# zhaoshan2/pangu-pytorch

Hardware: AMD Instinct MI355X
Metric: forward steps/sec (721x1440x13pl) per MI355X (higher is better)
Workload: dtype f32; 1 GPU; PanguModel fp32 forward, 1 sample/GPU, input (1,5,13,721,1440)+(1,4,721,1440), depths 2-6-6-2, dims 192/384, random-init weights (BASELINE configs[1]); parallelism=dp1

## Files before the change

### include/pangu_hip.h

```cpp
#ifndef PANGU_HIP_H
#define PANGU_HIP_H

#include <stdint.h>

#ifdef __cplusplus
extern "C" {
#endif

#define PANGU_ABI_VERSION 1

#define PANGU_OK 0
#define PANGU_E_SHAPE (-1)
#define PANGU_E_NULL (-2)
#define PANGU_E_DTYPE (-3)
#define PANGU_E_ARG (-4)
#define PANGU_E_RANGE (-5)

#define PANGU_F32 0
#define PANGU_BF16 1

#define PANGU_ACT_NONE 0
#define PANGU_ACT_GELU 1
#define PANGU_ACT_GELU_BWD 2
#define PANGU_ACT_ADD 3
#define PANGU_ACT_GELU_BWD_H 4

typedef void* pangu_stream_t;

int pangu_abi_version(void);
const char* pangu_error_string(int code);


int pangu_window_index_export(pangu_stream_t stream, int32_t* out, int Z, int H, int W, int shifted);

int pangu_window_mask_export(pangu_stream_t stream, float* out, int Z, int H, int W);


int pangu_linear_fwd(pangu_stream_t stream, const float* A, int lda, const float* W, const float* bias,
                     float* C, int ldc, int M, int N, int K, int act, float* aux);

int pangu_split_weight_bf16x3(pangu_stream_t stream, const float* W, int N, int K, void* image);
int pangu_linear_fwd_split(pangu_stream_t stream, const float* A, int lda, const void* image, const float* bias,
                           float* C, int ldc, int M, int N, int K, int act);

int pangu_linear_wgrad(pangu_stream_t stream, const float* dC, int lddc, const float* A, int lda, float* dW,
                       float* db, int M, int N, int K);
int pangu_linear_wgrad_ws(pangu_stream_t stream, const float* dC, int lddc, const float* A, int lda, float* dW,
                          float* db, int M, int N, int K, float* workspace, long long workspace_bytes);


int pangu_lora_wgrad_f32(pangu_stream_t stream, const float* dY, int lddy, const float* X, int ldx, const float* A,
                         const float* B, float* dA, float* dB, int M, int N, int K, int r, float scaling, float* workspace,
                         long long workspace_bytes);
int pangu_lora_wgrad_bf16(pangu_stream_t stream, const void* dY, int lddy, const void* X, int ldx, const float* A, const float* B,
                          float* dA, float* dB, int M, int N, int K, int r, float scaling, float* workspace,
                          long long workspace_bytes);
int pangu_lora_merge_f32(pangu_stream_t stream, const float* W, const float* A, const float* B, float* W_eff, int N, int K,
                         int r, float scaling);


int pangu_lora_dropout_fwd_f32(pangu_stream_t stream, const float* X, int ldx, float* Y, int ldy, const float* A, const float* B,
                               int M, int N, int K, int r, float scaling, double p, unsigned seed, int act, float* H, int ldh);
int pangu_lora_wgrad_dropout_f32(pangu_stream_t stream, const float* dY, int lddy, const float* X, int ldx, const float* A,
                                 const float* B, float* dA, float* dB, float* V, int M, int N, int K, int r, float scaling, double p,
                                 unsigned seed, float* workspace, long long workspace_bytes);
int pangu_lora_dropout_dx_f32(pangu_stream_t stream, float* dX, int lddx, const float* V, const float* A, int M, int K, int r,
                              double p, unsigned seed, const float* pre, int ldpre);


int pangu_lora_dropout_fwd_bf16(pangu_stream_t stream, const void* X, int ldx, void* Y, int ldy, const float* A, const float* B,
                                int M, int N, int K, int r, float scaling, double p, unsigned seed, int act, void* H, int ldh);
int pangu_lora_wgrad_dropout_bf16(pangu_stream_t stream, const void* dY, int lddy, const void* X, int ldx, const float* A,
                                  const float* B, float* dA, float* dB, float* V, int M, int N, int K, int r, float scaling, double p,
                                  unsigned seed, float* workspace, long long workspace_bytes);
int pangu_lora_dropout_dx_bf16(pangu_stream_t stream, void* dX, int lddx, const float* V, const float* A, int M, int K, int r,
                               double p, unsigned seed, const void* pre, int ldpre);


int pangu_window_attn_fwd(pangu_stream_t stream, const float* qkv, const float* qkv_bias, const float* esb,
                          float* out, float* lse, int Z, int H, int W, int C, int heads, int shifted);
int pangu_window_attn_fwd_compact(pangu_stream_t stream, const float* qkv, const float* qkv_bias,
                                  const float* esb_compact, float* out, float* lse, int Z, int H, int W, int C,
                                  int heads, int shifted);

int pangu_attn_windows_fwd(pangu_stream_t stream, const float* qkv, const float* esb, const float* mask,
                           long long mask_lon_stride, float* out, int n_lon, int types, int heads, int C);

int pangu_attn_windows_bwd(pangu_stream_t stream, const float* qkv, const float* esb, const float* mask,
                           long long mask_lon_stride, const float* dout, float* dqkv, float* d_esb, int n_lon, int types,
                           int heads, int C);

int pangu_window_attn_bwd(pangu_stream_t stream, const float* qkv, const float* qkv_bias, const float* esb,
                          const float* out, const float* lse, const float* dout, float* dqkv, float* dqkv_bias,
                          float* d_esb, int Z, int H, int W, int C, int heads, int shifted);


int pangu_ln_residual_fwd(pangu_stream_t stream, const float* y, const float* shortcut, int lds,
                          const float* gamma, const float* beta, float* out, int ldo, float* mean_rstd,
                          int N, int C, float branch_scale);

int pangu_linear_ln_residual_fwd(pangu_stream_t stream, const float* A, int lda, const float* W, const float* bias,
                                 const float* shortcut, int lds, const float* gamma, const float* beta, float* out, int ldo,
                                 int M, int N, int K, float branch_scale);

int pangu_linear_ln_residual_fwd_split(pangu_stream_t stream, const float* A, int lda, const void* image, const float* bias,
                                       const float* shortcut, int lds, const float* gamma, const float* beta, float* out,
                                       int ldo, int M, int N, int K, float branch_scale);

int pangu_ln_residual_bwd(pangu_stream_t stream, const float* dout, int lddo, const float* y, const float* gamma,
                          float* dy, float* dgamma, float* dbeta, int N, int C, float branch_scale);

int pangu_downsample_ln_fwd(pangu_stream_t stream, const float* x, int ldx, const float* gamma,
                            const float* beta, float* out, float* mean_rstd, int Z, int H, int W, int C);

int pangu_downsample_ln_bwd(pangu_stream_t stream, const float* dout, const float* x, int ldx, const float* gamma,
                            float* dx, float* dgamma, float* dbeta, int Z, int H, int W, int C, const float* dx_add);

int pangu_upsample_ln_fwd(pangu_stream_t stream, const float* y, const float* gamma, const float* beta,
                          float* out, float* mean_rstd, int Z, int H2, int W2, int H, int Co);

int pangu_upsample_ln_bwd(pangu_stream_t stream, const float* dout, const float* y, const float* gamma, float* dy,
                          float* dgamma, float* dbeta, int Z, int H2, int W2, int H, int Co);


int pangu_patch_embed_gather(pangu_stream_t stream, const float* input, const float* input_surface,
                             const float* surface_mean, const float* surface_std, const float* upper_mean,
                             const float* upper_std, const float* maps, const float* const_h,
                             float* a_surface, float* a_upper, int LAT, int LON, int levels_reversed);

int pangu_patch_embed_gather_bwd(pangu_stream_t stream, const float* da_surface, const float* da_upper,
                                 const float* surface_std, const float* upper_std, float* d_input,
                                 float* d_input_surface, int LAT, int LON, int levels_reversed);

int pangu_patch_recover_scatter(pangu_stream_t stream, const float* y_upper, const float* y_surface,
                                float* output, float* output_surface, int LAT, int LON);
int pangu_patch_recover_scatter_denorm(pangu_stream_t stream, const float* y_upper, const float* y_surface, float* output,
                                       float* output_surface, float* phys, float* phys_surface, const float* upper_mean,
                                       const float* upper_std, const float* surface_mean, const float* surface_std, int LAT,
                                       int LON);

int pangu_patch_recover_gather_bwd(pangu_stream_t stream, const float* d_output, const float* d_output_surface,
                                   float* dy_upper, float* dy_surface, int LAT, int LON);


int pangu_lat_weighted_sums(pangu_stream_t stream, const float* pred, const float* target, const float* lat_weight,
                            float* out, int planes, int H, int W);


int pangu_ensemble_perturb_f32(pangu_stream_t stream, float* upper, long long upper_member_stride, float* surface,
                               long long surface_member_stride, int E, int first_member, int H, int W, const float* amplitude,
                               const float* upper_std, const float* surface_std, unsigned int seed, int octaves, int period,
                               float persistence, int control);

int pangu_ensemble_stats_f32(pangu_stream_t stream, const float* members, long long member_stride, int E, const float* target,
                             const float* clim, const float* lat_weight, float* out, float* mean_out, float* std_out,
                             float* workspace, long long workspace_bytes, int planes, int H, int W);

int pangu_ensemble_reliability_f32(pangu_stream_t stream, const float* members, long long member_stride, int E,
                                   const float* target, const float* thresholds, int T, const float* lat_weight,
                                   unsigned int seed, int first_plane, unsigned int* counts, float* freq, float* prob,
                                   void* workspace, long long workspace_bytes, int planes, int H, int W);

long long pangu_ensemble_quantiles_ws_bytes(int planes, int H, int Q);
int pangu_ensemble_quantiles_f32(pangu_stream_t stream, const float* members, long long member_stride, int E,
                                 const double* levels, int Q, const float* target, const float* lat_weight, float* fields,
                                 float* pinball, unsigned int* coverage_count, float* coverage_freq, unsigned int* nonfinite,
// ... 139 lines not shown
```

### pangu-pytorch_amd/_lib.py

```python
import ctypes
import os
import re

_HERE = os.path.dirname(os.path.abspath(__file__))
LIB_PATH = os.environ.get("PANGU_HIP_LIB") or os.path.join(_HERE, "libpangu_hip.so")
HEADER_PATH = os.path.join(os.path.dirname(_HERE), "include", "pangu_hip.h")

_c = ctypes
_P, _I, _F = _c.c_void_p, _c.c_int, _c.c_float

SIGNATURES = {
    "pangu_abi_version": [],
    "pangu_error_string": [_I],
    "pangu_window_index_export": [_P, _P, _I, _I, _I, _I],
    "pangu_window_mask_export": [_P, _P, _I, _I, _I],
    "pangu_linear_fwd": [_P, _P, _I, _P, _P, _P, _I, _I, _I, _I, _I, _P],
    "pangu_split_weight_bf16x3": [_P, _P, _I, _I, _P],
    "pangu_linear_fwd_split": [_P, _P, _I, _P, _P, _P, _I, _I, _I, _I, _I],
    "pangu_linear_wgrad": [_P, _P, _I, _P, _I, _P, _P, _I, _I, _I],
    "pangu_linear_wgrad_ws": [_P, _P, _I, _P, _I, _P, _P, _I, _I, _I, _P, _c.c_longlong],
    "pangu_lora_wgrad_f32": [_P, _P, _I, _P, _I, _P, _P, _P, _P, _I, _I, _I, _I, _F, _P, _c.c_longlong],
    "pangu_lora_wgrad_bf16": [_P, _P, _I, _P, _I, _P, _P, _P, _P, _I, _I, _I, _I, _F, _P, _c.c_longlong],
    "pangu_lora_merge_f32": [_P, _P, _P, _P, _P, _I, _I, _I, _F],
    "pangu_lora_dropout_fwd_f32": [_P, _P, _I, _P, _I, _P, _P, _I, _I, _I, _I, _F, _c.c_double, _c.c_uint, _I, _P, _I],
    "pangu_lora_wgrad_dropout_f32": [_P, _P, _I, _P, _I, _P, _P, _P, _P, _P, _I, _I, _I, _I, _F, _c.c_double, _c.c_uint, _P,
                                     _c.c_longlong],
    "pangu_lora_dropout_dx_f32": [_P, _P, _I, _P, _P, _I, _I, _I, _c.c_double, _c.c_uint, _P, _I],
    "pangu_lora_dropout_fwd_bf16": [_P, _P, _I, _P, _I, _P, _P, _I, _I, _I, _I, _F, _c.c_double, _c.c_uint, _I, _P, _I],
    "pangu_lora_wgrad_dropout_bf16": [_P, _P, _I, _P, _I, _P, _P, _P, _P, _P, _I, _I, _I, _I, _F, _c.c_double, _c.c_uint, _P,
                                      _c.c_longlong],
    "pangu_lora_dropout_dx_bf16": [_P, _P, _I, _P, _P, _I, _I, _I, _c.c_double, _c.c_uint, _P, _I],
    "pangu_window_attn_bwd": [_P] * 10 + [_I] * 6,
    "pangu_ln_residual_bwd": [_P, _P, _I, _P, _P, _P, _P, _P, _I, _I, _F],
    "pangu_downsample_ln_bwd": [_P, _P, _P, _I, _P, _P, _P, _P, _I, _I, _I, _I, _P],
    "pangu_upsample_ln_bwd": [_P, _P, _P, _P, _P, _P, _P, _I, _I, _I, _I, _I],
    "pangu_patch_recover_gather_bwd": [_P, _P, _P, _P, _P, _I, _I],
    "pangu_lat_weighted_sums": [_P, _P, _P, _P, _P, _I, _I, _I],
    "pangu_ensemble_perturb_f32": [_P, _P, _c.c_longlong, _P, _c.c_longlong, _I, _I, _I, _I, _P, _P, _P, _c.c_uint, _I, _I, _F, _I],
    "pangu_ensemble_stats_f32": [_P, _P, _c.c_longlong, _I, _P, _P, _P, _P, _P, _P, _P, _c.c_longlong, _I, _I, _I],
    "pangu_ensemble_reliability_f32": [_P, _P, _c.c_longlong, _I, _P, _P, _I, _P, _c.c_uint, _I, _P, _P, _P, _P, _c.c_longlong, _I, _I,
                                       _I],
    "pangu_ensemble_quantiles_ws_bytes": [_I, _I, _I],
    "pangu_ensemble_quantiles_f32": [_P, _P, _c.c_longlong, _I, _P, _I, _P, _P, _P, _P, _P, _P, _P, _P, _c.c_longlong, _I, _I, _I],
    "pangu_zonal_spectrum_ws_bytes": [_I, _I, _I, _I, _I],
    "pangu_zonal_spectrum_f32": [_P, _P, _c.c_longlong, _I, _P, _P, _I, _P, _P, _I, _P, _P, _c.c_longlong, _I, _I, _I],
    "pangu_linear_fwd_bf16": [_P, _P, _I, _P, _P, _P, _I, _I, _I, _I, _I, _P, _I],
    "pangu_window_attn_fwd_bf16": [_P, _P, _P, _P, _P, _P, _I, _I, _I, _I, _I, _I],
    "pangu_window_attn_qkv_fwd_bf16": [_P, _P, _I, _P, _P, _P, _P, _P, _I, _I, _I, _I, _I, _I],
    "pangu_ln_residual_fwd_bf16": [_P, _P, _P, _I, _P, _P, _P, _I, _I, _I, _F],
    "pangu_linear_ln_residual_fwd_bf16": [_P, _P, _I, _P, _P, _P, _P, _P, _P, _I, _I, _I, _I],
    "pangu_mlp_ln_residual_fwd_bf16": [_P, _P, _I, _P, _P, _P, _P, _P, _P, _I, _I, _I, _F],
    "pangu_mlp_ln_residual_train_fwd_bf16": [_P, _P, _I, _P, _P, _P, _P, _P, _P, _I, _P, _I, _P, _I, _I, _I, _F],
    "pangu_linear_gelu_bwd_bf16": [_P, _P, _I, _P, _P, _I, _I, _I, _I, _P, _P],
    "pangu_downsample_ln_fwd_bf16": [_P, _P, _I, _P, _P, _P, _I, _I, _I, _I],
    "pangu_upsample_ln_fwd_bf16": [_P, _P, _P, _P, _P, _I, _I, _I, _I, _I],
    "pangu_patch_embed_gather_bf16": [_P] * 11 + [_I, _I, _I],
    "pangu_linear_wgrad_bf16": [_P, _P, _I, _P, _I, _P, _P, _I, _I, _I],
    "pangu_linear_wgrad_bf16_ws": [_P, _P, _I, _P, _I, _P, _P, _I, _I, _I, _P, _c.c_longlong],
    "pangu_shadow_refresh_bf16": [_P, _P, _I, _c.c_longlong],
    "pangu_adam_step_multi": [_P, _P, _I, _c.c_longlong] + [_c.c_double] * 5 + [_F, _F],
    "pangu_grad_sumsq_multi": [_P, _P, _I, _c.c_longlong, _P],
    "pangu_grad_clip_state": [_P, _P, _c.c_longlong, _P, _I, _c.c_double, _c.c_double, _I],
    "pangu_adam_step_multi_scaled": [_P, _P, _I, _c.c_longlong] + [_c.c_double] * 5 + [_F, _F, _P],
    "pangu_weighted_l1_loss_blocks": [_I, _I, _c.c_longlong, _I, _c.c_longlong, _I],
    "pangu_weighted_l1_loss_fwd": [_P] * 9 + [_I, _I, _c.c_longlong, _I, _c.c_longlong, _I, _I] + [_P] * 4,
    "pangu_weighted_l1_loss_bwd": [_P] * 10 + [_I, _I, _c.c_longlong, _I, _c.c_longlong, _I, _I] + [_P] * 4,
    "pangu_rollout_l1_seed_bwd": [_P] * 14 + [_I, _I, _c.c_longlong, _I, _c.c_longlong, _I, _I] + [_P] * 4,
    "pangu_fair_crps_loss_blocks": [_I] * 7,
    "pangu_fair_crps_loss_fwd": [_P, _P, _P, _I] + [_P] * 7 + [_I] * 7 + [_P] * 4,
    "pangu_fair_crps_loss_bwd": [_P, _P, _P, _I] + [_P] * 8 + [_I] * 7 + [_P] * 4,
    "pangu_host_copy": [_P, _P, _c.c_longlong, _I],
    "pangu_pack_i16_ws_bytes": [_I, _c.c_longlong],
    "pangu_pack_planes_i16": [_P, _P, _P, _P, _P, _P, _P, _P, _c.c_longlong, _I, _c.c_longlong, _I],
    "pangu_stage_planes_f32": [_P, _P, _P, _P, _P, _I, _c.c_longlong, _I],
    "pangu_unpack_i16_host": [_P, _P, _P, _I, _c.c_longlong, _I],
    "pangu_regrid_planes_f32": [_P, _P, _P, _P, _P, _I, _I, _I, _I, _I, _P, _P, _P, _I, _P, _P, _P, _I, _I],
    "pangu_scorecard_ws_bytes": [_I, _I, _I],
    "pangu_scorecard_sums_f32": [_P, _P, _P, _I, _P, _I, _P, _P, _I, _P, _P, _c.c_longlong, _I, _I, _I],
    "pangu_event_scores_ws_bytes": [_I, _I, _I, _I],
    "pangu_event_scores_f32": [_P, _P, _P, _I, _P, _I, _P, _I, _P, _P, _I, _P, _P, _P, _P, _c.c_longlong, _I, _I, _I],
    "pangu_lead_stats_update_f32": [_P] * 10 + [_I, _P, _P, _P, _I, _c.c_longlong, _I, _I, _I],
    "pangu_window_attn_bwd_bf16": [_P] * 10 + [_I] * 6,
    "pangu_ln_residual_bwd_bf16": [_P, _P, _I, _P, _P, _P, _P, _P, _I, _I, _F],
    "pangu_downsample_ln_bwd_bf16": [_P, _P, _P, _I, _P, _P, _P, _P, _I, _I, _I, _I, _P],
    "pangu_upsample_ln_bwd_bf16": [_P, _P, _P, _P, _P, _P, _P, _I, _I, _I, _I, _I],
    "pangu_patch_recover_gather_bwd_bf16": [_P, _P, _P, _P, _P, _I, _I],
    "pangu_window_attn_fwd": [_P, _P, _P, _P, _P, _P, _I, _I, _I, _I, _I, _I],
    "pangu_window_attn_fwd_compact": [_P, _P, _P, _P, _P, _P, _I, _I, _I, _I, _I, _I],
    "pangu_attn_windows_fwd": [_P, _P, _P, _P, _c.c_longlong, _P, _I, _I, _I, _I],
    "pangu_attn_windows_bwd": [_P, _P, _P, _P, _c.c_longlong, _P, _P, _P, _I, _I, _I, _I],
    "pangu_ln_residual_fwd": [_P, _P, _P, _I, _P, _P, _P, _I, _P, _I, _I, _F],
    "pangu_linear_ln_residual_fwd": [_P, _P, _I, _P, _P, _P, _I, _P, _P, _P, _I, _I, _I, _I, _F],
    "pangu_linear_ln_residual_fwd_split": [_P, _P, _I, _P, _P, _P, _I, _P, _P, _P, _I, _I, _I, _I, _F],
    "pangu_downsample_ln_fwd": [_P, _P, _I, _P, _P, _P, _P, _I, _I, _I, _I],
    "pangu_upsample_ln_fwd": [_P, _P, _P, _P, _P, _P, _I, _I, _I, _I, _I],
    "pangu_patch_embed_gather": [_P] * 11 + [_I, _I, _I],
    "pangu_patch_embed_gather_bwd": [_P] * 7 + [_I, _I, _I],
    "pangu_patch_recover_scatter": [_P, _P, _P, _P, _P, _I, _I],
    "pangu_patch_recover_scatter_denorm": [_P] * 11 + [_I, _I],
    "pangu_traffic_copy": [_P, _P, _P, _c.c_longlong, _I],
}
_RESTYPES = {"pangu_error_string": _c.c_char_p, "pangu_weighted_l1_loss_blocks": _c.c_longlong,
             "pangu_fair_crps_loss_blocks": _c.c_longlong, "pangu_pack_i16_ws_bytes": _c.c_longlong,
             "pangu_ensemble_quantiles_ws_bytes": _c.c_longlong, "pangu_zonal_spectrum_ws_bytes": _c.c_longlong,
             "pangu_scorecard_ws_bytes": _c.c_longlong, "pangu_event_scores_ws_bytes": _c.c_longlong}

_lib = None


def header_functions():
    src = open(HEADER_PATH).read()
    src = re.sub(r"/\*.*?\*/", "", src, flags=re.S)
    return sorted(set(re.findall(r"\b(pangu_[a-z0-9_]+)\s*\(", src)))


def load():
    global _lib
    if _lib is not None:
        return _lib
    if not os.path.exists(LIB_PATH):
        raise RuntimeError(
            f"{LIB_PATH} not found: the HIP extension is not built. Run `python -c 'import __graft_entry__ as g; "
            "g.build()'` (or `make -C pangu-pytorch_amd/csrc`). There is no CPU fallback for this path.")
    import torch
    lib = ctypes.CDLL(LIB_PATH)
    for name, argtypes in SIGNATURES.items():
        fn = getattr(lib, name)
        fn.argtypes = argtypes
        fn.restype = _RESTYPES.get(name, _I)
    if lib.pangu_abi_version() != 1:
        raise RuntimeError("libpangu_hip.so ABI version mismatch")
    _lib = lib
    return lib


def check(rc, what):
    if rc != 0:
        msg = load().pangu_error_string(rc)
        raise RuntimeError(f"{what} failed: {msg.decode() if msg else rc} (code {rc})")
```

### pangu-pytorch_amd/fused.py

```python
import torch

from . import ops, ops_bf16 as ob
from .autograd import DownSampleFn, EarthBlockFn, MlpFn, PatchEmbedFn, PatchRecoverFn, PatchRecoverHalvesFn, UpSampleFn
from . import layers as _layers


def _train_path(module, *tensors):
    if not torch.is_grad_enabled():
        return False
    return any(p.requires_grad for p in module.parameters()) or any(t.requires_grad for t in tensors)


def _stack(outs, B):
    return outs[0].unsqueeze(0) if B == 1 else torch.stack(outs, 0)


def _samples(x):
    if x.shape[0] == 1:
        t = x.reshape(x.shape[1:])
        return [t if t.stride(-1) == 1 and t.dim() == 2 else t.contiguous()]
    return [t.contiguous() for t in x.unbind(0)]


def _tok2d(x):
    B, N, C = x.shape
    if x.stride(2) != 1 or (B > 1 and x.stride(0) != N * x.stride(1)):
        x = x.contiguous()
    return x.as_strided((B * N, C), (x.stride(1), 1), x.storage_offset())


def drop_path_scales(blk):
    dp = blk.drop_path
    if not hasattr(dp, "sample_scale"):
        return 1.0, 1.0
    return dp.sample_scale(blk.training), dp.sample_scale(blk.training)


def embed_constants(statistics, maps, const_h, LAT, LON, dev):
    f32 = lambda t: t.to(device=dev, dtype=torch.float32).contiguous()
    s_mean, s_std, u_mean, u_std = statistics
    return (f32(s_mean).reshape(-1), f32(s_std).reshape(-1), f32(u_mean).reshape(13, 5), f32(u_std).reshape(13, 5),
            f32(maps).reshape(3, 4 * ((LAT + 3) // 4), LON), f32(const_h).reshape(13, LAT, LON))


def concat_halves(x):
    N, C = x.shape[-2:]
    cat = torch.empty((N, 2 * C), dtype=x.dtype, device=x.device)
    return [torch.empty(0, dtype=x.dtype, device=x.device).set_(cat.untyped_storage(), cat.storage_offset() + off, (N, C), (2 * C, 1))
            for off in (0, C)]


def mlp(m, x2d):
    if _train_path(m, x2d) or _drops(m):
        return MlpFn.apply(x2d.contiguous(), _layers.eff_weight(m.linear1), m.linear1.bias, _layers.eff_weight(m.linear2),
                           m.linear2.bias, *_layers.lora_args(m.linear1, m.linear2))
    h = ops.linear(x2d, _layers.eff_weight(m.linear1), m.linear1.bias, act=ops.ACT_GELU)
    return ops.linear(h, _layers.eff_weight(m.linear2), m.linear2.bias)


def _plain_proj(blk, lin, x2, act=ops.ACT_NONE):
    w = _layers.eff_weight(lin)
    if getattr(blk, "split_projections", True):
        image = ops.split_image(lin, w, None if w is lin.weight else ("lora",) + tuple(lin._stamp()))
        if image is not None:
            return ops.linear_split(x2, image, w.shape[0], lin.bias, act=act)
    return ops.linear(x2, w, lin.bias, act=act)


_LN_SPLIT_NOT_DISPATCHED = {(384, 384)}


def _ln_proj(blk, lin, x2, shortcut, norm, out=None, branch_scale=1.0):
    w = _layers.eff_weight(lin)
    if getattr(blk, "split_projections", True) and tuple(w.shape) not in _LN_SPLIT_NOT_DISPATCHED:
        image = ops.split_image(lin, w, None if w is lin.weight else ("lora",) + tuple(lin._stamp()))
        if image is not None:
            return ops.linear_ln_residual_split(x2, image, w.shape[0], lin.bias, shortcut, norm.weight, norm.bias, out=out,
                                                branch_scale=branch_scale)
    return ops.linear_ln_residual(x2, w, lin.bias, shortcut, norm.weight, norm.bias, out=out, branch_scale=branch_scale)


def _block_rows(blk, x2, B, Z, H, W, roll, out=None):
    N, C = x2.shape[0] // B, x2.shape[1]
    att = blk.attention
    s1, s2 = drop_path_scales(blk)
    if s1 != 0.0:
        qkv = _plain_proj(blk, att.linear1, x2)
        esb_c = getattr(att, "_esb_compact", None)
        if esb_c is not None:
            p = att.earth_specific_bias
            if getattr(att, "_esb_compact_stamp", None) != ops.param_stamp(p) or esb_c.device != p.device:
                att._esb_compact = esb_c = None
        cp = esb_c is not None
        esb = esb_c if cp else att.earth_specific_bias[0]
        o = torch.cat([ops.window_attention(qkv[b * N:(b + 1) * N], att.linear1.bias, esb, Z, H, W,
                                            att.head_number, roll, compact=cp) for b in range(B)], 0) if B > 1 else \
            ops.window_attention(qkv, att.linear1.bias, esb, Z, H, W, att.head_number, roll, compact=cp)
        if C in (192, 384):
            x1 = _ln_proj(blk, att.linear2, o, x2, blk.norm1, branch_scale=s1)
        else:
            y = ops.linear(o, _layers.eff_weight(att.linear2), att.linear2.bias)
            x1 = ops.ln_residual(y, x2, blk.norm1.weight, blk.norm1.bias, branch_scale=s1)
    else:
        x1 = x2
    if s2 == 0.0:
        return x1 if out is None else out.copy_(x1)
    if C in (192, 384):
        h = _plain_proj(blk, blk.linear.linear1, x1, act=ops.ACT_GELU)
        return _ln_proj(blk, blk.linear.linear2, h, x1, blk.norm2, out=out, branch_scale=s2)
    return ops.ln_residual(mlp(blk.linear, x1), x1, blk.norm2.weight, blk.norm2.bias, out=out, branch_scale=s2)


def _block_rows_bf16(blk, sh, x, Z, H, W, roll, out=None):
    att = blk.attention
    s1, s2 = drop_path_scales(blk)
    C = x.shape[1]
    fuse_proj = x.is_contiguous() and s1 == 1.0 and s2 == 1.0 and C in (192, 384)
    if s1 != 0.0:
        if C in (192, 384):
            o = ob.window_attention_qkv(x, sh.get_lin(att.linear1), att.linear1.bias, sh.get(att.earth_specific_bias),
                                        Z, H, W, att.head_number, roll)
        else:
            qkv = ob.linear(x, sh.get_lin(att.linear1), att.linear1.bias)
            o = ob.window_attention(qkv, sh.get(att.linear1.bias), sh.get(att.earth_specific_bias), Z, H, W,
                                    att.head_number, roll)
        if fuse_proj:
            x1 = ob.linear_ln_residual(o, sh.get_lin(att.linear2), att.linear2.bias, x, blk.norm1.weight, blk.norm1.bias)
        else:
            y = ob.linear(o, sh.get_lin(att.linear2), att.linear2.bias)
            x1 = ob.ln_residual(y, x, blk.norm1.weight, blk.norm1.bias, branch_scale=s1)
    else:
        x1 = x
    if s2 == 0.0:
        return x1 if out is None else out.copy_(x1)
    if C in (192, 384):
        return ob.mlp_ln_residual(x1, sh.get_mlp_lin(blk.linear.linear1, blk.linear.linear2),
                                  blk.linear.linear1.bias, blk.linear.linear2.bias, blk.norm2.weight, blk.norm2.bias,
                                  out=out, branch_scale=s2)
    h = ob.linear(x1, sh.get_lin(blk.linear.linear1), blk.linear.linear1.bias, act=ob.ACT_GELU)
    m = ob.linear(h, sh.get_lin(blk.linear.linear2), blk.linear.linear2.bias)
    return ob.ln_residual(m, x1, blk.norm2.weight, blk.norm2.bias, out=out, branch_scale=s2)


def _drops(layer):
    return layer.training and _layers.dropout_active(layer)


def _infer_arm(layer, sh, infer, *tensors):
    if sh is not None:
        if infer and _drops(layer):
            raise RuntimeError("LoRA adapter dropout in a bf16 train()-mode forward runs on the gradient path only (the inference "
                               "kernels have no materialised projections to correct): call eval() first")
        return infer
    return not (_train_path(layer, *tensors) or _drops(layer))


def sample_block(blk, x, Z, H, W, roll, out=None, sh=None, infer=False):
    if _infer_arm(blk, sh, infer, x):
        return _block_rows(blk, x, 1, Z, H, W, roll, out) if sh is None else _block_rows_bf16(blk, sh, x, Z, H, W, roll, out)
    att = blk.attention
    s1, s2 = drop_path_scales(blk)
    return EarthBlockFn.apply(
        x, blk.norm1.weight, blk.norm1.bias, blk.norm2.weight, blk.norm2.bias,
        _layers.eff_weight(blk.linear.linear1), blk.linear.linear1.bias,
        _layers.eff_weight(blk.linear.linear2), blk.linear.linear2.bias, att.earth_specific_bias,
        _layers.eff_weight(att.linear1), att.linear1.bias, _layers.eff_weight(att.linear2), att.linear2.bias,
        (Z, H, W, att.head_number, bool(roll)), s1, s2, None if out is None else (out,), sh,
        *_layers.lora_args(blk.linear.linear1, blk.linear.linear2, att.linear1, att.linear2))


def _embed_rows(m, inp, inp_surface, consts, levels_reversed, out):
    a_s, a_u = ops.patch_embed_gather(inp, inp_surface, *consts, levels_reversed)
    n_s = a_s.shape[0]
    ops.linear(a_s, m.conv_surface.weight, m.conv_surface.bias, out=out[:n_s])
    ops.linear(a_u, m.conv.weight, m.conv.bias, out=out[n_s:])
    return out


def sample_embed(m, inp, inp_surface, consts, levels_reversed=False, sh=None):
    if sh is None and not _train_path(m, inp, inp_surface):
# ... 115 lines not shown
```

### pangu-pytorch_amd/ops.py

```python
import threading
import weakref

import torch

from . import _lib

ACT_NONE, ACT_GELU, ACT_GELU_BWD, ACT_ADD = 0, 1, 2, 3

_timing = None


def timing_start():
    global _timing
    _timing = []


def timing_stop(kind, also=()):
    global _timing
    rec, _timing = _timing or [], None
    torch.cuda.synchronize()

    def agg(tag):
        sel = [(a.elapsed_time(b), w) for k, a, b, w in rec if k == tag]
        return sum(t for t, _ in sel), sum(w for _, w in sel), len(sel)
# ... 419 lines not shown
        raise RuntimeError(f"lora_wgrad: dy {tuple(dy.shape)} x {tuple(x.shape)} A {tuple(A.shape)} B {tuple(B.shape)}")
    ws = wgrad_workspace(dy.device)
    dA = torch.empty((r, K), dtype=torch.float32, device=dy.device)
    dB = torch.empty((N, r), dtype=torch.float32, device=dy.device)
    with _timed("lora_wgrad", 4.0 * M * (K + N)):
        _lib.check(lib.pangu_lora_wgrad_f32(_stream(dy), dp, lddy, xp, ldx, _chk(A, "lora_A"), _chk(B, "lora_B"), dA.data_ptr(),
                                            dB.data_ptr(), M, N, K, r, float(scaling), ws.data_ptr(), _WGRAD_WS_BYTES), "lora_wgrad")
    return dA, dB


def _lora_shapes(what, x, y, A, B):
    M, N = y.shape
    K = x.shape[1]
    r = A.shape[0]
    if x.shape[0] != M or tuple(A.shape) != (r, K) or tuple(B.shape) != (N, r):
        raise RuntimeError(f"{what}: y {tuple(y.shape)} x {tuple(x.shape)} A {tuple(A.shape)} B {tuple(B.shape)}")
    return M, N, K, r


def lora_dropout_fwd(x, y, A, B, scaling, p, seed, act=ACT_NONE, h=None):
    lib = _lib.load()
    xp, ldx = _rows(x, "lora_dropout_fwd.x")
    yp, ldy = _rows(y, "lora_dropout_fwd.y")
    M, N, K, r = _lora_shapes("lora_dropout_fwd", x, y, A, B)
    if act not in (ACT_NONE, ACT_GELU):
        raise RuntimeError(f"lora_dropout_fwd: act {act} (ACT_NONE or ACT_GELU)")
    hp, ldh = (None, 0)
    if act == ACT_GELU:
        if h is None:
            h = torch.empty((M, N), dtype=torch.float32, device=y.device)
        if tuple(h.shape) != (M, N):
            raise RuntimeError(f"lora_dropout_fwd: h {tuple(h.shape)} != {(M, N)}")
        hp, ldh = _rows(h, "lora_dropout_fwd.h")
    with _timed("lora_dropout_fwd", 4.0 * M * (K + 2 * N + (N if act == ACT_GELU else 0))):
        _lib.check(lib.pangu_lora_dropout_fwd_f32(_stream(y), xp, ldx, yp, ldy, _chk(A, "lora_A"), _chk(B, "lora_B"), M, N, K, r,
                                                  float(scaling), float(p), int(seed), act, hp, ldh), "lora_dropout_fwd")
    return (y, h) if act == ACT_GELU else y


def lora_wgrad_dropout(dy, x, A, B, scaling, p, seed):
    lib = _lib.load()
    dp, lddy = _rows(dy, "lora_wgrad_dropout.dy")
    xp, ldx = _rows(x, "lora_wgrad_dropout.x")
    M, N, K, r = _lora_shapes("lora_wgrad_dropout", x, dy, A, B)
    ws = wgrad_workspace(dy.device)
    dA = torch.empty((r, K), dtype=torch.float32, device=dy.device)
    dB = torch.empty((N, r), dtype=torch.float32, device=dy.device)
    V = torch.empty((M, r), dtype=torch.float32, device=dy.device)
    with _timed("lora_wgrad_dropout", 4.0 * M * (K + N + r)):
        _lib.check(lib.pangu_lora_wgrad_dropout_f32(_stream(dy), dp, lddy, xp, ldx, _chk(A, "lora_A"), _chk(B, "lora_B"),
                                                    dA.data_ptr(), dB.data_ptr(), V.data_ptr(), M, N, K, r, float(scaling), float(p),
                                                    int(seed), ws.data_ptr(), _WGRAD_WS_BYTES), "lora_wgrad_dropout")
    return dA, dB, V


def lora_dropout_dx(dx, V, A, p, seed, pre=None):
    lib = _lib.load()
    xp, lddx = _rows(dx, "lora_dropout_dx.dx")
    M, K = dx.shape
    r = A.shape[0]
    if tuple(V.shape) != (M, r) or tuple(A.shape) != (r, K) or (pre is not None and tuple(pre.shape) != (M, K)):
        raise RuntimeError(f"lora_dropout_dx: dx {tuple(dx.shape)} V {tuple(V.shape)} A {tuple(A.shape)}")
    pp, ldp = _rows(pre, "lora_dropout_dx.pre") if pre is not None else (None, 0)
    with _timed("lora_dropout_dx", 4.0 * M * (2 * K + r + (K if pre is not None else 0))):
        _lib.check(lib.pangu_lora_dropout_dx_f32(_stream(dx), xp, lddx, _chk(V, "lora_V"), _chk(A, "lora_A"), M, K, r, float(p),
                                                 int(seed), pp, ldp), "lora_dropout_dx")
    return dx


def lora_merge(W, A, B, scaling, out=None):
    lib = _lib.load()
    W2 = W.reshape(W.shape[0], -1)
    N, K = W2.shape
    r = A.shape[0]
    if tuple(A.shape) != (r, K) or tuple(B.shape) != (N, r):
        raise RuntimeError(f"lora_merge: W {tuple(W.shape)} A {tuple(A.shape)} B {tuple(B.shape)}")
    if out is None:
        out = torch.empty((N, K), dtype=torch.float32, device=W.device)
    _lib.check(lib.pangu_lora_merge_f32(_stream(W), _chk(W2, "weight"), _chk(A, "lora_A"), _chk(B, "lora_B"), _chk(out, "W_eff"),
                                        N, K, r, float(scaling)), "lora_merge")
    return out


def window_attention(qkv, qkv_bias, esb, Z, H, W, heads, shifted, want_lse=False, compact=False):
    lib = _lib.load()
    N, C3 = qkv.shape
    C = C3 // 3
    if N != Z * H * W:
        raise RuntimeError(f"window_attention: {N} tokens != {Z}x{H}x{W}")
    types = (Z // 2) * ((H + 5) // 6)
    want = (types, heads, 3312) if compact else (types, heads, 144, 144)
    if tuple(esb.shape) != want:
        raise RuntimeError(f"window_attention: bias table {tuple(esb.shape)} != {want}")
    out = torch.empty((N, C), dtype=torch.float32, device=qkv.device)
    lse = torch.empty((N, heads), dtype=torch.float32, device=qkv.device) if want_lse else None
    Np = (Z // 2) * ((H + 5) // 6) * (W // 12) * 144
    with _timed("attn", 4.0 * Np * 144 * C):
        fn = lib.pangu_window_attn_fwd_compact if compact else lib.pangu_window_attn_fwd
        _lib.check(fn(_stream(qkv), _chk(qkv, "qkv"), _chk(qkv_bias, "qkv_bias"), _chk(esb, "esb"), out.data_ptr(),
                      lse.data_ptr() if want_lse else None, Z, H, W, C, heads, int(shifted)), "window_attn_fwd")
    return (out, lse) if want_lse else out


def attention_windows(qkv, esb, mask, n_lon, types, heads):
    lib = _lib.load()
    M, C3 = qkv.shape
    C = C3 // 3
    if M != n_lon * types * 144 or tuple(esb.shape) != (types, heads, 144, 144):
        raise RuntimeError(f"attention_windows: qkv {tuple(qkv.shape)}, esb {tuple(esb.shape)} vs {n_lon} x {types} windows")
    stride = 0
    if mask is not None:
        if tuple(mask.shape) == (n_lon, types, 144, 144):
            stride = types * 144 * 144
        elif tuple(mask.shape) != (types, 144, 144):
            raise RuntimeError(f"attention_windows: mask {tuple(mask.shape)} is neither ({n_lon}, {types}, 144, 144) nor ({types}, 144, 144)")
    out = torch.empty((M, C), dtype=torch.float32, device=qkv.device)
    _lib.check(lib.pangu_attn_windows_fwd(_stream(qkv), _chk(qkv, "qkv"), _chk(esb, "esb"),
                                          _chk(mask, "mask") if mask is not None else None, stride, out.data_ptr(), n_lon, types,
                                          heads, C), "attn_windows_fwd")
    return out


def attention_windows_bwd(qkv, esb, mask, dout, n_lon, types, heads):
    lib = _lib.load()
    M, C3 = qkv.shape
    C = C3 // 3
    if M != n_lon * types * 144 or tuple(esb.shape) != (types, heads, 144, 144) or tuple(dout.shape) != (M, C):
        raise RuntimeError(f"attention_windows_bwd: qkv {tuple(qkv.shape)}, esb {tuple(esb.shape)}, dout {tuple(dout.shape)}")
    stride = 0
    if mask is not None:
        if tuple(mask.shape) == (n_lon, types, 144, 144):
            stride = types * 144 * 144
        elif tuple(mask.shape) != (types, 144, 144):
            raise RuntimeError(f"attention_windows_bwd: mask {tuple(mask.shape)}")
    dqkv = torch.empty_like(qkv)
    desb = torch.empty_like(esb)
    _lib.check(lib.pangu_attn_windows_bwd(_stream(qkv), _chk(qkv, "qkv"), _chk(esb, "esb"),
                                          _chk(mask, "mask") if mask is not None else None, stride, _chk(dout, "dout"),
                                          dqkv.data_ptr(), desb.data_ptr(), n_lon, types, heads, C), "attn_windows_bwd")
    return dqkv, desb


def window_attention_bwd(qkv, qkv_bias, esb, out, lse, dout, Z, H, W, heads, shifted, desb_out=None):
    lib = _lib.load()
    N, C3 = qkv.shape
    C = C3 // 3
    dqkv = torch.empty_like(qkv)
    dqb = _zeros((C3,), qkv.device)
    desb = torch.empty_like(esb) if desb_out is None else desb_out.view(esb.shape)
    Np = (Z // 2) * ((H + 5) // 6) * (W // 12) * 144
    with _timed("attn_bwd", 14.0 * Np * 144 * C):
        _lib.check(lib.pangu_window_attn_bwd(_stream(qkv), _chk(qkv, "qkv"), _chk(qkv_bias, "qkv_bias"), _chk(esb, "esb"),
                                             _chk(out, "out"), _chk(lse, "lse"), _chk(dout, "dout"), dqkv.data_ptr(),
                                             dqb.data_ptr(), desb.data_ptr(), Z, H, W, C, heads, int(shifted)),
                   "window_attn_bwd")
    return dqkv, dqb, desb


def ln_residual_bwd(dout, y, gamma, branch_scale=1.0):
    lib = _lib.load()
    N, C = y.shape
    dp, lddo = _rows(dout, "ln_bwd.dout")
    dy = torch.empty_like(y)
    dg, db = _zeros((2, C), y.device).unbind(0)
    _lib.check(lib.pangu_ln_residual_bwd(_stream(dout), dp, lddo, _chk(y, "ln_bwd.y"), _chk(gamma, "gamma"), dy.data_ptr(),
                                         dg.data_ptr(), db.data_ptr(), N, C, float(branch_scale)), "ln_residual_bwd")
    return dy, dg, db


def downsample_ln_bwd(dout, x, gamma, Z, H, W, add=None):
    lib = _lib.load()
    xp, ldx = _rows(x, "downsample_bwd.x")
    C = x.shape[1]
    dx = torch.empty((Z * H * W, C), dtype=torch.float32, device=x.device)
    if add is not None and tuple(add.shape) != tuple(dx.shape):
        raise RuntimeError(f"downsample_ln_bwd: addend {tuple(add.shape)} != {tuple(dx.shape)}")
    dg, db = _zeros((2, 4 * C), x.device).unbind(0)
    _lib.check(lib.pangu_downsample_ln_bwd(_stream(dout), _chk(dout, "dout"), xp, ldx, _chk(gamma, "gamma"), dx.data_ptr(),
                                           dg.data_ptr(), db.data_ptr(), Z, H, W, C,
                                           _chk(add, "downsample_bwd.add") if add is not None else None), "downsample_ln_bwd")
# ... 134 lines not shown
```

Before: 20.23 forward steps/s.

## Add bf16x3 split-precision MFMA window attention kernel for fp32 inference

Adds a new fp32 window-attention forward kernel that splits Q, K, V and probabilities into three bf16 components and runs the QK^T and PV products on bf16 MFMA instructions with six partial products, keeping near-fp32 accuracy. It is dispatched by default for inference through a new split flag, replacing the previous fp32 attention path. The same change also enables the split linear+LN residual path for the 384x384 shape. The cost is six times as many MFMA ops plus splitting overhead and no lse output, traded against the much higher bf16 matrix throughput compared with fp32 arithmetic.

```diff
diff --git a/include/pangu_hip.h b/include/pangu_hip.h
--- a/include/pangu_hip.h
+++ b/include/pangu_hip.h
@@ -82,6 +82,11 @@
 int pangu_window_attn_fwd_compact(pangu_stream_t stream, const float* qkv, const float* qkv_bias,
                                   const float* esb_compact, float* out, float* lse, int Z, int H, int W, int C,
                                   int heads, int shifted);
+int pangu_window_attn_fwd_split(pangu_stream_t stream, const float* qkv, const float* qkv_bias, const float* esb,
+                                float* out, int Z, int H, int W, int C, int heads, int shifted);
+int pangu_window_attn_fwd_split_compact(pangu_stream_t stream, const float* qkv, const float* qkv_bias,
+                                        const float* esb_compact, float* out, int Z, int H, int W, int C, int heads,
+                                        int shifted);
 
 int pangu_attn_windows_fwd(pangu_stream_t stream, const float* qkv, const float* esb, const float* mask,
                            long long mask_lon_stride, float* out, int n_lon, int types, int heads, int C);
diff --git a/pangu-pytorch_amd/_lib.py b/pangu-pytorch_amd/_lib.py
--- a/pangu-pytorch_amd/_lib.py
+++ b/pangu-pytorch_amd/_lib.py
@@ -87,6 +87,8 @@
     "pangu_patch_recover_gather_bwd_bf16": [_P, _P, _P, _P, _P, _I, _I],
     "pangu_window_attn_fwd": [_P, _P, _P, _P, _P, _P, _I, _I, _I, _I, _I, _I],
     "pangu_window_attn_fwd_compact": [_P, _P, _P, _P, _P, _P, _I, _I, _I, _I, _I, _I],
+    "pangu_window_attn_fwd_split": [_P, _P, _P, _P, _P, _I, _I, _I, _I, _I, _I],
+    "pangu_window_attn_fwd_split_compact": [_P, _P, _P, _P, _P, _I, _I, _I, _I, _I, _I],
     "pangu_attn_windows_fwd": [_P, _P, _P, _P, _c.c_longlong, _P, _I, _I, _I, _I],
     "pangu_attn_windows_bwd": [_P, _P, _P, _P, _c.c_longlong, _P, _P, _P, _I, _I, _I, _I],
     "pangu_ln_residual_fwd": [_P, _P, _P, _I, _P, _P, _P, _I, _P, _I, _I, _F],
diff --git a/pangu-pytorch_amd/csrc/attn_f32_split.hip b/pangu-pytorch_amd/csrc/attn_f32_split.hip
--- /dev/null
+++ b/pangu-pytorch_amd/csrc/attn_f32_split.hip
@@ -0,0 +1,318 @@
+#include "common.h"
+
+#include "attn_bf16_tile.h"
+#include "split_f32.h"
+
+namespace {
+
+constexpr int KPLANE = PANGU_WTOK * 64;
+constexpr int VPLANE = 32 * 256;
+
+__device__ inline int vt128_off(int d, int key) { return d * 256 + ((((key >> 3) ^ d) & 15) << 4) + (key & 7) * 2; }
+constexpr int NW = 3, NT = 64 * NW, TPW = 9 / NW;
+constexpr int UPT = 576 / NT;
+static_assert(3 * (3 * KPLANE + 3 * VPLANE) <= 160 * 1024, "three workgroups per CU");
+
+typedef f32x4 f32x4_al4 __attribute__((aligned(4)));
+constexpr int COMPACT_BIAS = 3312;
+
+template <bool COMPACT>
+__device__ __forceinline__ void load_bias_row_il(f32x4 (&s)[9], const float* __restrict__ bias_tile, int qn, int lg) {
+  if (COMPACT) {
+    const int zq = qn / 72, hq = (qn / 12) % 6, wq = qn % 12;
+#pragma unroll
+    for (int j = 0; j < 9; ++j) {
+      const int k0 = key_of(j, 4 * lg);
+      const int zk = k0 / 72, hk = (k0 / 12) % 6, wk = k0 % 12;
+      const int idx = (zq + 2 * zk) * 828 + (hq + 6 * hk) * 23 + (wq - wk + 11);
+      const f32x4 v = *reinterpret_cast<const f32x4_al4*>(bias_tile + idx - 3);
+      s[j] = f32x4{v[3], v[2], v[1], v[0]};
+    }
+  } else {
+    const float* brow = bias_tile + (size_t)qn * PANGU_WTOK;
+#pragma unroll
+    for (int j = 0; j < 9; ++j) s[j] = *reinterpret_cast<const f32x4*>(brow + key_of(j, 4 * lg));
+  }
+}
+
+typedef short bf16x4s __attribute__((ext_vector_type(4)));
+
+#define PANGU_SPLIT6(MFMA, acc, ah, am, al, bh, bm, bl) \
+  do {                                                  \
+    acc = MFMA(al, bh, acc, 0, 0, 0);                   \
+    acc = MFMA(ah, bl, acc, 0, 0, 0);                   \
+    acc = MFMA(am, bm, acc, 0, 0, 0);                   \
+    acc = MFMA(am, bh, acc, 0, 0, 0);                   \
+    acc = MFMA(ah, bm, acc, 0, 0, 0);                   \
+    acc = MFMA(ah, bh, acc, 0, 0, 0);                   \
+  } while (0)
+
+template <bool SHIFTED>
+__device__ __forceinline__ void split_tile(const unsigned char* Kp, const unsigned char* Vp, const f32x4 q0, const f32x4 q1,
+                                           f32x4 (&s)[9], int qn, int qtok, int lq, int lg, bool zcut, bool hcut,
+                                           unsigned long long kz_bits, unsigned long long kh_bits,
+                                           const bf16x4s (&vtail)[2][3], float* __restrict__ out, int C, int hd) {
+  int ke = kswz(key_of(0, lq), lg), kt = kswz(128 + lq, lg);
+  int vrow = lq * 256, vx = ((lg ^ lq) & 15) << 4;
+  asm volatile("" : "+v"(ke), "+v"(kt), "+v"(vrow), "+v"(vx));
+  const int ko = ke ^ 32;
+
+  bf16x8 qh, qm, ql;
+  pangu_split::split8(q0, q1, qh, qm, ql);
+#pragma unroll
+  for (int j0 = 0; j0 < 9; j0 += 3) {
+    bf16x8 kf[3][3];
+#pragma unroll
+    for (int jj = 0; jj < 3; ++jj) {
+      const int j = j0 + jj;
+      const int ka = j == 8 ? kt : ((j & 1) ? ko : ke) + 2048 * (j >> 1) + 256 * (j & 1);
+#pragma unroll
+      for (int p = 0; p < 3; ++p) kf[jj][p] = *reinterpret_cast<const bf16x8*>(Kp + p * KPLANE + ka);
+    }
+#define PANGU_S3(KP, QF)                                                                                              \
+  _Pragma("unroll") for (int jj = 0; jj < 3; ++jj) s[j0 + jj] =                                                       \
+      __builtin_amdgcn_mfma_f32_16x16x32_bf16(kf[jj][KP], QF, s[j0 + jj], 0, 0, 0)
+    PANGU_S3(2, qh);
+    PANGU_S3(0, ql);
+    PANGU_S3(1, qm);
+    PANGU_S3(1, qh);
+    PANGU_S3(0, qm);
+    PANGU_S3(0, qh);
+#undef PANGU_S3
+  }
+
+  float mx = -INFINITY;
+  if (SHIFTED) {
+    if (zcut || hcut) {
+      const bool zq = qn >= 72, hq = ((qn / 12) % 6) < 3;
+      const unsigned long long zsel = zq ? ~kz_bits : kz_bits;
+      const unsigned long long hsel = hq ? ~kh_bits : kh_bits;
+      const unsigned long long cut = (zcut ? zsel : 0ull) | (hcut ? hsel : 0ull);
+#pragma unroll
+      for (int j = 0; j < 9; ++j)
+#pragma unroll
+        for (int r = 0; r < 4; ++r)
+          if ((cut >> (4 * j + r)) & 1ull) s[j][r] += -100.0f;
+    }
+  }
+#pragma unroll
+  for (int j = 0; j < 9; ++j)
+#pragma unroll
+    for (int r = 0; r < 4; ++r) mx = fmaxf(mx, s[j][r]);
+  mx = fmaxf(mx, __shfl_xor(mx, 16, 64));
+  mx = fmaxf(mx, __shfl_xor(mx, 32, 64));
+  float sum = 0.f;
+  const float nmx = -mx * 1.4426950408889634f;
+#pragma unroll
+  for (int j = 0; j < 9; ++j)
+#pragma unroll
+    for (int r = 0; r < 4; ++r) {
+      const float e = __builtin_amdgcn_exp2f(fmaf(s[j][r], 1.4426950408889634f, nmx));
+      s[j][r] = e;
+      sum += e;
+    }
+  sum += __shfl_xor(sum, 16, 64);
+  sum += __shfl_xor(sum, 32, 64);
+
+  f32x4 o0 = {0.f, 0.f, 0.f, 0.f}, o1 = {0.f, 0.f, 0.f, 0.f};
+#pragma unroll
+  for (int u = 0; u < 4; ++u) {
+    bf16x8 ph, pm, pl, v0[3], v1[3];
+    const int a0 = vrow + (vx ^ (64 * u)), a1 = a0 + 16 * 256;
+#pragma unroll
+    for (int p = 0; p < 3; ++p) {
+      v0[p] = *reinterpret_cast<const bf16x8*>(Vp + p * VPLANE + a0);
+      v1[p] = *reinterpret_cast<const bf16x8*>(Vp + p * VPLANE + a1);
+    }
+    pangu_split::split8(s[2 * u], s[2 * u + 1], ph, pm, pl);
+#define PANGU_O2(VP, PF)                                                    \
+  o0 = __builtin_amdgcn_mfma_f32_16x16x32_bf16(v0[VP], PF, o0, 0, 0, 0);    \
+  o1 = __builtin_amdgcn_mfma_f32_16x16x32_bf16(v1[VP], PF, o1, 0, 0, 0)
+    PANGU_O2(2, ph);
+    PANGU_O2(0, pl);
+    PANGU_O2(1, pm);
+    PANGU_O2(1, ph);
+    PANGU_O2(0, pm);
+    PANGU_O2(0, ph);
+#undef PANGU_O2
+  }
+  {
+    unsigned h0, h1, m0, m1, l0, l1;
+    pangu_split::split2(s[8][0], s[8][1], h0, m0, l0);
+    pangu_split::split2(s[8][2], s[8][3], h1, m1, l1);
+    const bf16x4s ph = __builtin_bit_cast(bf16x4s, u32x2{h0, h1}), pm = __builtin_bit_cast(bf16x4s, u32x2{m0, m1}),
+                  pl = __builtin_bit_cast(bf16x4s, u32x2{l0, l1});
+    PANGU_SPLIT6(__builtin_amdgcn_mfma_f32_16x16x16bf16_1k, o0, vtail[0][0], vtail[0][1], vtail[0][2], ph, pm, pl);
+    PANGU_SPLIT6(__builtin_amdgcn_mfma_f32_16x16x16bf16_1k, o1, vtail[1][0], vtail[1][1], vtail[1][2], ph, pm, pl);
+  }
+
+  if (qtok >= 0) {
+    const float inv = 1.0f / sum;
+    float* dst = out + (size_t)qtok * C + hd * 32 + lg * 4;
+    *reinterpret_cast<f32x4*>(dst) = o0 * inv;
+    *reinterpret_cast<f32x4*>(dst + 16) = o1 * inv;
+  }
+}
+
+template <bool SHIFTED, bool COMPACT>
+__global__ __launch_bounds__(NT, 3) void window_attn_f32_split_kernel(const float* __restrict__ qkv,
+                                                                         const float* __restrict__ qkv_bias,
+                                                                         const float* __restrict__ esb, float* __restrict__ out,
+                                                                         WinGeom g, int C, int heads, int n_pairs) {
+  __shared__ __attribute__((aligned(16))) unsigned char Kp[3 * KPLANE];
+  __shared__ __attribute__((aligned(16))) unsigned char Vp[3 * VPLANE];
+
+  const int b = blockIdx.x;
+  const int xcd = b & 7, local = b >> 3;
+  const int pair = (local / g.nLon) * 8 + xcd;
+  const int l = local % g.nLon;
+  if (pair >= n_pairs) return;
+  const int t = pair / heads, hd = pair - t * heads;
+
+  const int tid = threadIdx.x, lane = tid & 63, wave = tid >> 6;
+  const int lq = lane & 15, lg = lane >> 4;
+  const int C3 = 3 * C;
+  const float scale = 0.17677669529663687f;
+  const float* bias_tile = esb + (size_t)(t * heads + hd) * (COMPACT ? COMPACT_BIAS : PANGU_WTOK * PANGU_WTOK);
+
+  f32x4 k0[UPT], k1[UPT], va[UPT], vb[UPT];
+#pragma unroll
+  for (int i = 0; i < UPT; ++i) {
+    const int f = tid + NT * i;
+    {
+      const int tok = win_src_token(g, l, t, f >> 2, SHIFTED);
+      const float* src = (tok >= 0 ? qkv + (size_t)tok * C3 : qkv_bias) + C + hd * 32 + (f & 3) * 8;
+      k0[i] = *reinterpret_cast<const f32x4*>(src);
+      k1[i] = *reinterpret_cast<const f32x4*>(src + 4);
+    }
+    {
+      const int n = 2 * (f >> 3), c = (f & 7) * 4;
+      if (n < 128) {
+        const int ta = win_src_token(g, l, t, n, SHIFTED), tb = win_src_token(g, l, t, n + 1, SHIFTED);
+        va[i] = *reinterpret_cast<const f32x4*>((ta >= 0 ? qkv + (size_t)ta * C3 : qkv_bias) + 2 * C + hd * 32 + c);
+        vb[i] = *reinterpret_cast<const f32x4*>((tb >= 0 ? qkv + (size_t)tb * C3 : qkv_bias) + 2 * C + hd * 32 + c);
+      }
+    }
+  }
+  int qtok[TPW];
+  f32x4 q0[TPW], q1[TPW];
+#pragma unroll
+  for (int i = 0; i < TPW; ++i) {
+    const int qn = (wave + NW * i) * 16 + lq;
+    qtok[i] = win_src_token(g, l, t, qn, SHIFTED);
+    const float* src = (qtok[i] >= 0 ? qkv + (size_t)qtok[i] * C3 : qkv_bias) + hd * 32 + lg * 8;
+    q0[i] = *reinterpret_cast<const f32x4*>(src);
+    q1[i] = *reinterpret_cast<const f32x4*>(src + 4);
+  }
+  float vta[2][4];
+#pragma unroll
+  for (int r = 0; r < 4; ++r) {
+    const int tok = win_src_token(g, l, t, 128 + 4 * lg + r, SHIFTED);
+    const float* src = (tok >= 0 ? qkv + (size_t)tok * C3 : qkv_bias) + 2 * C + hd * 32 + lq;
+    vta[0][r] = src[0];
+    vta[1][r] = src[16];
+  }
+
+  bool zcut = false, hcut = false;
+  unsigned long long kz_bits = 0ull, kh_bits = 0ull;
+  if (SHIFTED) {
+    const int zwin = t / g.nHw, hwin = t - zwin * g.nHw;
+    zcut = zwin == g.nZw - 1;
+    hcut = hwin == g.nHw - 1;
+#pragma unroll
+    for (int j = 0; j < 9; ++j)
+#pragma unroll
+      for (int r = 0; r < 4; ++r) {
+        const int kn = key_of(j, lg * 4 + r);
+        if (kn >= 72) kz_bits |= 1ull << (4 * j + r);
+        if (((kn / 12) % 6) < 3) kh_bits |= 1ull << (4 * j + r);
+      }
+  }
+
+#pragma unroll
+  for (int i = 0; i < UPT; ++i) {
+    const int f = tid + NT * i;
+    bf16x8 h, m, lo;
+    pangu_split::split8(k0[i], k1[i], h, m, lo);
+    const int ka = kswz(f >> 2, f & 3);
+    *reinterpret_cast<bf16x8*>(Kp + ka) = h;
+    *reinterpret_cast<bf16x8*>(Kp + KPLANE + ka) = m;
+    *reinterpret_cast<bf16x8*>(Kp + 2 * KPLANE + ka) = lo;
+    const int n = 2 * (f >> 3), c = (f & 7) * 4;
+    if (n < 128) {
+#pragma unroll
+      for (int e = 0; e < 4; ++e) {
+        unsigned vh, vm, vl;
+        pangu_split::split2(va[i][e], vb[i][e], vh, vm, vl);
+        const int a = vt128_off(c + e, n);
+        *reinterpret_cast<unsigned*>(Vp + a) = vh;
+        *reinterpret_cast<unsigned*>(Vp + VPLANE + a) = vm;
+        *reinterpret_cast<unsigned*>(Vp + 2 * VPLANE + a) = vl;
+      }
+    }
+  }
+  bf16x4s vtail[2][3];
+#pragma unroll
+  for (int dt = 0; dt < 2; ++dt) {
+    unsigned h0, h1, m0, m1, l0, l1;
+    pangu_split::split2(vta[dt][0], vta[dt][1], h0, m0, l0);
+    pangu_split::split2(vta[dt][2], vta[dt][3], h1, m1, l1);
+    vtail[dt][0] = __builtin_bit_cast(bf16x4s, u32x2{h0, h1});
+    vtail[dt][1] = __builtin_bit_cast(bf16x4s, u32x2{m0, m1});
+    vtail[dt][2] = __builtin_bit_cast(bf16x4s, u32x2{l0, l1});
+  }
+#pragma unroll
+  for (int i = 0; i < TPW; ++i) { q0[i] *= scale; q1[i] *= scale; }
+  f32x4 sA[9], sB[9];
+  load_bias_row_il<COMPACT>(sA, bias_tile, wave * 16 + lq, lg);
+  __syncthreads();
+
+#pragma unroll
+  for (int i = 0; i < TPW; ++i) {
+    f32x4 (&sc)[9] = (i & 1) ? sB : sA;
+    f32x4 (&sn)[9] = (i & 1) ? sA : sB;
+    if (i + 1 < TPW) load_bias_row_il<COMPACT>(sn, bias_tile, (wave + NW * (i + 1)) * 16 + lq, lg);
+    split_tile<SHIFTED>(Kp, Vp, q0[i], q1[i], sc, (wave + NW * i) * 16 + lq, qtok[i], lq, lg, zcut, hcut, kz_bits, kh_bits,
+                        vtail, out, C, hd);
+  }
+}
+
+int check_split_geom(int Z, int H, int W) {
+  if (Z <= 0 || H <= 0 || W <= 0) return PANGU_E_SHAPE;
+  if (Z % PANGU_WZ || (H + PANGU_PAD_H) % PANGU_WH || W % PANGU_WW) return PANGU_E_SHAPE;
+  return PANGU_OK;
+}
+
+}
+
+static int launch_attn_split(pangu_stream_t stream, const float* qkv, const float* qkv_bias, const float* esb, float* out,
+                             int Z, int H, int W, int C, int heads, int shifted, bool compact) {
+  if (!qkv || !qkv_bias || !esb || !out) return PANGU_E_NULL;
+  if (int e = check_split_geom(Z, H, W)) return e;
+  if (heads <= 0 || C != heads * PANGU_HEAD_DIM) return PANGU_E_SHAPE;
+  const WinGeom g = make_geom(Z, H, W);
+  const int n_pairs = g.types * heads;
+  const int grid = ((n_pairs + 7) / 8) * 8 * g.nLon;
+  hipStream_t s = (hipStream_t)stream;
+#define PANGU_LAUNCH_ATTN(SH, CP)                                                                                       \
+  hipLaunchKernelGGL((window_attn_f32_split_kernel<SH, CP>), dim3(grid), dim3(NT), 0, s, qkv, qkv_bias, esb, out, g, C, heads, \
+                     n_pairs)
+  if (shifted) {
+    if (compact) PANGU_LAUNCH_ATTN(true, true); else PANGU_LAUNCH_ATTN(true, false);
+  } else {
+    if (compact) PANGU_LAUNCH_ATTN(false, true); else PANGU_LAUNCH_ATTN(false, false);
+  }
+#undef PANGU_LAUNCH_ATTN
+  return pangu_launch_status();
+}
+
+extern "C" int pangu_window_attn_fwd_split(pangu_stream_t stream, const float* qkv, const float* qkv_bias, const float* esb,
+                                           float* out, int Z, int H, int W, int C, int heads, int shifted) {
+  return launch_attn_split(stream, qkv, qkv_bias, esb, out, Z, H, W, C, heads, shifted, false);
+}
+
+extern "C" int pangu_window_attn_fwd_split_compact(pangu_stream_t stream, const float* qkv, const float* qkv_bias,
+                                                   const float* esb_compact, float* out, int Z, int H, int W, int C, int heads,
+                                                   int shifted) {
+  return launch_attn_split(stream, qkv, qkv_bias, esb_compact, out, Z, H, W, C, heads, shifted, true);
+}
diff --git a/pangu-pytorch_amd/fused.py b/pangu-pytorch_amd/fused.py
--- a/pangu-pytorch_amd/fused.py
+++ b/pangu-pytorch_amd/fused.py
@@ -67,7 +67,7 @@
     return ops.linear(x2, w, lin.bias, act=act)
 
 
-_LN_SPLIT_NOT_DISPATCHED = {(384, 384)}
+_LN_SPLIT_NOT_DISPATCHED = set()
 
 
 def _ln_proj(blk, lin, x2, shortcut, norm, out=None, branch_scale=1.0):
@@ -78,6 +78,9 @@
             return ops.linear_ln_residual_split(x2, image, w.shape[0], lin.bias, shortcut, norm.weight, norm.bias, out=out,
                                                 branch_scale=branch_scale)
     return ops.linear_ln_residual(x2, w, lin.bias, shortcut, norm.weight, norm.bias, out=out, branch_scale=branch_scale)
+
+
+_ATTN_SPLIT_NOT_DISPATCHED = set()
 
 
 def _block_rows(blk, x2, B, Z, H, W, roll, out=None):
@@ -93,9 +96,10 @@
                 att._esb_compact = esb_c = None
         cp = esb_c is not None
         esb = esb_c if cp else att.earth_specific_bias[0]
+        sp = bool(getattr(blk, "split_projections", True)) and C not in _ATTN_SPLIT_NOT_DISPATCHED
         o = torch.cat([ops.window_attention(qkv[b * N:(b + 1) * N], att.linear1.bias, esb, Z, H, W,
-                                            att.head_number, roll, compact=cp) for b in range(B)], 0) if B > 1 else \
-            ops.window_attention(qkv, att.linear1.bias, esb, Z, H, W, att.head_number, roll, compact=cp)
+                                            att.head_number, roll, compact=cp, split=sp) for b in range(B)], 0) if B > 1 else \
+            ops.window_attention(qkv, att.linear1.bias, esb, Z, H, W, att.head_number, roll, compact=cp, split=sp)
         if C in (192, 384):
             x1 = _ln_proj(blk, att.linear2, o, x2, blk.norm1, branch_scale=s1)
         else:
diff --git a/pangu-pytorch_amd/ops.py b/pangu-pytorch_amd/ops.py
--- a/pangu-pytorch_amd/ops.py
+++ b/pangu-pytorch_amd/ops.py
@@ -525,8 +525,10 @@
     return out
 
 
-def window_attention(qkv, qkv_bias, esb, Z, H, W, heads, shifted, want_lse=False, compact=False):
-    lib = _lib.load()
+def window_attention(qkv, qkv_bias, esb, Z, H, W, heads, shifted, want_lse=False, compact=False, split=False):
+    lib = _lib.load()
+    if split and want_lse:
+        raise RuntimeError("window_attention: the exact-split kernel is inference only and produces no lse")
     N, C3 = qkv.shape
     C = C3 // 3
     if N != Z * H * W:
@@ -539,6 +541,11 @@
     lse = torch.empty((N, heads), dtype=torch.float32, device=qkv.device) if want_lse else None
     Np = (Z // 2) * ((H + 5) // 6) * (W // 12) * 144
     with _timed("attn", 4.0 * Np * 144 * C):
+        if split:
+            fn = lib.pangu_window_attn_fwd_split_compact if compact else lib.pangu_window_attn_fwd_split
+            _lib.check(fn(_stream(qkv), _chk(qkv, "qkv"), _chk(qkv_bias, "qkv_bias"), _chk(esb, "esb"), out.data_ptr(),
+                          Z, H, W, C, heads, int(shifted)), "window_attn_fwd_split")
+            return out
         fn = lib.pangu_window_attn_fwd_compact if compact else lib.pangu_window_attn_fwd
         _lib.check(fn(_stream(qkv), _chk(qkv, "qkv"), _chk(qkv_bias, "qkv_bias"), _chk(esb, "esb"), out.data_ptr(),
                       lse.data_ptr() if want_lse else None, Z, H, W, C, heads, int(shifted)), "window_attn_fwd")
```

New measurement: 21.30 forward steps/s, median of 6. 1.05x the previous value.
